# MegviiRobot/CamLaserCalibraTool

Measured on NVIDIA H100. Metric: residual+Jacobian evals/sec (full LM solves), higher is better.
Workload: dtype f64

## Files before the change

### camlasercalibratool_b200/_lib.py

```python
from __future__ import annotations

import ctypes as C
import os

from . import _build

c_double_p = C.POINTER(C.c_double)
c_int64_p = C.POINTER(C.c_int64)


class ClcError(RuntimeError):
    pass


class ProblemDesc(C.Structure):
    _fields_ = [
        ("n_frames", C.c_int64),
        ("frame_pose", c_double_p),
        ("offsets", c_int64_p),
        ("points", c_double_p),
        ("edge_points", c_double_p),
        ("use_loss", C.c_int),
        ("cauchy_a", C.c_double),
        ("device", C.c_int),
# ... 141 lines not shown
                                    C.POINTER(C.c_int32), C.POINTER(C.c_int32), C.c_int]),
    "clc_estimate_board_poses": (C.c_int, [C.POINTER(CameraDesc), C.c_int64, c_int64_p, C.POINTER(C.c_int32), C.POINTER(C.c_float),
                                           c_double_p, C.POINTER(C.c_int32), C.c_int]),
    "clc_T_to_pose7": (None, [c_double_p, c_double_p]),
    "clc_pose7_to_T": (None, [c_double_p, c_double_p]),
    "clc_shard_range": (C.c_int, [C.c_int64, c_int64_p, C.c_int, C.c_int, c_int64_p, c_int64_p]),
    "clc_comm_unique_id": (C.c_int, [_P]),
    "clc_comm_create": (C.c_int, [C.POINTER(_P), _P, C.c_int, C.c_int, C.c_int]),
    "clc_comm_destroy": (C.c_int, [_P]),
    "clc_comm_p2p_export": (C.c_int, [_P, _P]),
    "clc_comm_p2p_import": (C.c_int, [_P, _P]),
    "clc_problem_attach_comm": (C.c_int, [_P, _P]),
    "clc_problem_set_allreduce_mode": (C.c_int, [_P, C.c_int]),
    "clc_bench_eval": (C.c_int, [_P, c_double_p, C.c_int, C.c_int, C.POINTER(C.c_float)]),
    "clc_problem_algorithmic_bytes": (C.c_int, [_P, c_int64_p]),
    "clc_problem_streamed_bytes": (C.c_int, [_P, c_int64_p]),
    "clc_problem_set_planar_mode": (C.c_int, [_P, C.c_int]),
    "clc_debug_pack": (C.c_int, [C.c_int64, C.POINTER(c_double_p), c_int64_p, C.c_int64, C.c_int64, C.c_int, c_double_p,
                                 C.POINTER(C.c_int)]),
    "clc_debug_partition": (C.c_int, [_P, C.POINTER(C.c_int), c_int64_p, C.POINTER(C.c_int), C.POINTER(C.c_int),
                                      C.POINTER(C.c_int)]),
    "clc_debug_dispatch": (C.c_int, [_P, C.POINTER(C.c_int), C.POINTER(C.c_int), C.POINTER(C.c_int), C.POINTER(C.c_int),
                                     C.POINTER(C.c_int)]),
    "clc_bench_h2d": (C.c_int, [C.c_int64, C.c_int, C.c_int, C.POINTER(C.c_float)]),
    "clc_solve_readback_bytes": (C.c_int64, []),
    "clc_host_alloc": (C.c_int, [C.POINTER(_P), C.c_int64]),
    "clc_host_free": (C.c_int, [_P]),
    "clc_launch_count": (C.c_int64, []),
}

_lib = None


def lib_path() -> str:
    return _build.LIB_PATH


def load():
    global _lib
    if _lib is not None:
        return _lib
    path = os.environ.get("CLC_LIB_PATH", _build.LIB_PATH)
    if path == _build.LIB_PATH and _build.is_stale():
        try:
            _build.build()
        except Exception as exc:
# ... 19 lines not shown
```

### camlasercalibratool_b200/api.py

```python
from __future__ import annotations

import ctypes as C
from dataclasses import dataclass, field

import numpy as np

from . import _lib
from ._lib import ClcError, GatherDesc, LmIteration, LmOptions, LmSummary, ProblemDesc, SyntheticDesc, TERMINATION


def _dp(a):
    return a.ctypes.data_as(_lib.c_double_p) if a is not None else None


def _ip(a):
    return a.ctypes.data_as(_lib.c_int64_p) if a is not None else None


@dataclass
class Oberserve:

    tagPose_Qca: np.ndarray = field(default_factory=lambda: np.array([0.0, 0.0, 0.0, 1.0]))
    tagPose_tca: np.ndarray = field(default_factory=lambda: np.zeros(3))
    points: np.ndarray = field(default_factory=lambda: np.zeros((0, 3)))
# ... 59 lines not shown
    d.n_frames_total = int(n_frames_total)
    d.frame_begin = int(frame_begin)
    d.frame_end = int(n_frames_total if frame_end is None else frame_end)
    d.beams, d.seed, d.sigma = int(beams), int(seed), float(sigma)
    d.with_edges, d.use_loss, d.cauchy_a, d.device = int(bool(with_edges)), int(bool(use_loss)), float(cauchy_a), int(device)
    d.camera_model = {None: 0, "none": 0, "radtan": 1, "pinhole": 1, "equi": 2}[camera]
    if d.camera_model:
        k = CAMERA_DEFAULTS["radtan" if d.camera_model == 1 else "equi"] if intrinsics is None else intrinsics
        d.camera_intrinsics = (C.c_double * 8)(*[float(v) for v in k])
        d.pixel_sigma = float(pixel_sigma)
        d.image_width, d.image_height = int(image_size[0]), int(image_size[1])
        d.grid_rows, d.grid_cols, d.tag_size, d.tag_spacing = int(grid[0]), int(grid[1]), float(grid[2]), float(grid[3])
    return d


def default_options(**kw) -> LmOptions:
    o = LmOptions()
    _lib.load().clc_lm_default_options(C.byref(o))
    for k, v in kw.items():
        setattr(o, k, v)
    return o


class Problem:

    def __init__(self, handle):
        self._h = handle
        self._L = _lib.load()
        self._comm = None

    @classmethod
    def from_arrays(cls, frame_pose, offsets, points, edge_points=None, use_loss=True, cauchy_a=0.05, device=-1):
        L = _lib.load()
        frame_pose = np.ascontiguousarray(frame_pose, dtype=np.float64).reshape(-1, 7)
        offsets = np.ascontiguousarray(offsets, dtype=np.int64)
        points = np.ascontiguousarray(points, dtype=np.float64).reshape(-1, 3)
        if edge_points is not None:
            edge_points = np.ascontiguousarray(edge_points, dtype=np.float64).reshape(-1, 6)
            if edge_points.shape[0] != frame_pose.shape[0]:
                raise ValueError("edge_points must be [n_frames, 6]")
        if offsets.shape[0] != frame_pose.shape[0] + 1 or (offsets.size and offsets[-1] != points.shape[0]):
            raise ValueError("offsets do not match frame_pose / points")
        d = ProblemDesc()
        d.n_frames = frame_pose.shape[0]
        d.frame_pose, d.offsets, d.points, d.edge_points = _dp(frame_pose), _ip(offsets), _dp(points), _dp(edge_points)
        d.use_loss, d.cauchy_a, d.device = int(bool(use_loss)), float(cauchy_a), int(device)
# ... 55 lines not shown
        b = C.c_int64()
        _lib.check(self._L.clc_problem_streamed_bytes(self._h, C.byref(b)), "clc_problem_streamed_bytes")
        return b.value

    @property
    def planar(self):
        return self.streamed_bytes() != self.algorithmic_bytes()

    def set_planar_mode(self, mode):
        _lib.check(self._L.clc_problem_set_planar_mode(self._h, int(mode)), "clc_problem_set_planar_mode")

    def partition(self, warp_table=True):
        grid, per_warp, stage, resident = C.c_int(), C.c_int64(), C.c_int(), C.c_int()
        L = self._L
        _lib.check(L.clc_debug_partition(self._h, C.byref(grid), C.byref(per_warp), C.byref(stage), C.byref(resident), None),
                   "clc_debug_partition")
        out = dict(grid=grid.value, per_warp=per_warp.value, stage=stage.value, resident_chunks=resident.value)
        if warp_table:
            wff = np.empty(grid.value * 12, dtype=np.int32)
            _lib.check(L.clc_debug_partition(self._h, None, None, None, None, wff.ctypes.data_as(C.POINTER(C.c_int))),
                       "clc_debug_partition")
            out["warp_first_frame"] = wff
        return out

    def dispatch(self):
        paths = [C.c_int() for _ in range(4)]
        shape = (C.c_int * 3)()
        _lib.check(self._L.clc_debug_dispatch(self._h, *[C.byref(v) for v in paths], shape), "clc_debug_dispatch")
        out = {k: _lib.PATHS[v.value] for k, v in zip(("eval", "information", "closed_form", "solve"), paths)}
        out["small_shape"] = tuple(shape)
        return out

    def download(self):
        nf, npts, he = self.sizes()
        fp, off, pts = np.empty((nf, 7)), np.empty(nf + 1, dtype=np.int64), np.empty((npts, 3))
        edge = np.empty((nf, 6)) if he else None
        planes = np.empty((nf, 4))
        _lib.check(self._L.clc_problem_download(self._h, _dp(fp), _ip(off), _dp(pts), _dp(edge), _dp(planes)),
                   "clc_problem_download")
        return dict(frame_pose=fp, offsets=off, points=pts, edge_points=edge, planes=planes)

    def download_true_poses(self):
        fp = np.empty((self.sizes()[0], 7))
        _lib.check(self._L.clc_problem_download_true_poses(self._h, _dp(fp)), "clc_problem_download_true_poses")
        return fp

# ... 288 lines not shown
```

### camlasercalibratool_b200/csrc/clc_api.cu

```cuda
#include <cuda_runtime.h>
#include <dlfcn.h>
#include <nccl.h>

#include <algorithm>
#include <atomic>
#include <chrono>
#include <cstdio>
#include <cstdlib>
#include <cstring>
#include <mutex>
#include <string>
#include <vector>

#include "../../include/clc_b200.h"
#include "clc_kernels.cuh"
#include "clc_l2_plan.h"
#include "clc_linefit.cuh"
#include "clc_small.cuh"

namespace {

thread_local std::string g_last_error;
std::atomic<int64_t> g_launches{0};

// ... 200 lines not shown
  int64_t l2_bytes = 0;
  int grid = 0;
  int64_t n_frames = 0, n_points = 0, n_points_padded = 0, n_edges = 0;
  int use_loss = 1;
  double cauchy_a = 0.05;
  double *x = nullptr, *y = nullptr, *z = nullptr;
  void *xy_block = nullptr, *z_block = nullptr;
  double* frame_pose = nullptr;
  double* frame_pose_true = nullptr;
  double* plane = nullptr;
  int64_t* offsets = nullptr;
  int* warp_first_frame = nullptr;
  double* edge_plane = nullptr;
  double* edge_pt = nullptr;
  unsigned long long* partials_ll = nullptr;
  unsigned int* launch_seq = nullptr;
  unsigned long long* pose_ll = nullptr;
  double* sums = nullptr;
  double* pose = nullptr;
  clc::LmState* lm = nullptr;
  double* flush_buf = nullptr;
  int64_t flush_n = 0;
  unsigned long long* timing = nullptr;
  bool use_pdl = true;
  int64_t l2_persist_bytes = 0;
  bool l2_window_set = false;
  int64_t l2_resident_bytes = -1;
  int resident_chunks = 0;
  bool small_kernel = true;
  int loop_in_kernel = 1;
  PinnedBlock* pinned = nullptr;
  double* h_sums = nullptr;
  int* h_done = nullptr;
  clc::LmState* h_lm = nullptr;
  clc_comm* comm_obj = nullptr;
  ncclComm_t comm = nullptr;
  int nranks = 1, rank = 0;
  int* p2p_error = nullptr;
  int allreduce_mode = 0;
  int64_t per_warp = 0;
  int grid_full = 0;
  cudaEvent_t ev0 = nullptr, ev1 = nullptr;
  int* d_nonplanar = nullptr;
  bool z_all_zero = false;
  bool host_planarity_known = false;
  bool planar = false;
  int planar_mode = 1;
  int64_t planar_min_points = 0;
};

namespace {

clc::ProblemView make_view(const clc_problem* p) {
  clc::ProblemView v;
  v.x = p->x; v.y = p->y; v.z = p->z;
  v.plane = p->plane;
  v.offsets = p->offsets;
  v.warp_first_frame = p->warp_first_frame;
  v.edge_plane = p->edge_plane;
  v.edge_pt = p->edge_pt;
  v.n_frames = p->n_frames;
  v.n_points = p->n_points;
  v.n_edges = p->n_edges;
  v.per_warp = p->per_warp;
  v.resident_chunks = p->resident_chunks;
  v.a2 = p->cauchy_a * p->cauchy_a;
  v.inv_a2 = 1.0 / v.a2;
  return v;
}

int set_device(const clc_problem* p) {
  CLC_CUDA(cudaSetDevice(p->device));
  return CLC_OK;
}

int launch_sweep(clc_problem* p, int mode, bool loss, bool edges, const double* d_pose, const int* d_done,
                 clc::LmState* d_lm, bool collective = true, bool pdl = false, int loop_sweeps = 1, bool l2_hints = false) {
  clc::SweepArgs a;
  a.pose7 = d_pose;
  a.done = d_done;
  a.partials_ll = p->partials_ll;
  a.sums = p->sums;
  a.launch_seq = p->launch_seq;
  a.pose_ll = p->pose_ll;
  a.lm = d_lm;
  a.use_loss = loss ? 1 : 0;
  a.use_edges = edges ? 1 : 0;
  a.l2_hints = l2_hints ? 1 : 0;
  a.loop_sweeps = loop_sweeps;
  a.timing = p->timing;
  a.nranks = 1;
  a.rank = 0;
  a.seq_counter = nullptr;
  a.error = p->p2p_error;
  if (p->nranks > 1 && p->allreduce_mode == 1 && collective) {
    clc_comm* c = p->comm_obj;
    a.nranks = c->nranks;
    a.rank = c->rank;
    a.seq_counter = reinterpret_cast<unsigned long long*>(static_cast<char*>(c->p2p_block) + c->mailbox_bytes());
    for (int r = 0; r < c->nranks; ++r) a.peer_mailbox[r] = static_cast<unsigned long long*>(c->peer_block[r]);
  }
  const clc::ProblemView v = make_view(p);
  cudaLaunchConfig_t cfg = {};
  cfg.gridDim = dim3((unsigned)p->grid);
  cfg.blockDim = dim3(clc::kThreads);
  cfg.dynamicSmemBytes = clc::dyn_smem_bytes(p->planar);
  cfg.stream = p->stream;
  cudaLaunchAttribute attr[1];
  attr[0].id = cudaLaunchAttributeProgrammaticStreamSerialization;
  attr[0].val.programmaticStreamSerializationAllowed = pdl ? 1 : 0;
  cfg.attrs = attr;
  cfg.numAttrs = 1;
  cudaError_t le;
// ... 56 lines not shown
  p->grid = p->grid_full;
  {
    const int64_t stages = (p->n_points + chunk - 1) / chunk;
    const int64_t blocks_needed = std::max<int64_t>(1, (stages + clc::kWarps - 1) / clc::kWarps);
    if (blocks_needed < p->grid) p->grid = (int)blocks_needed;
    int64_t single_block_max = (int64_t)clc::kWarps * 8 * clc::kChunk;
    if (const char* env = std::getenv("CLC_SINGLE_BLOCK_MAX_POINTS")) single_block_max = std::atoll(env);
    if (p->n_points <= single_block_max) p->grid = 1;
  }
  const int64_t n_warps = (int64_t)p->grid * clc::kWarps;
  p->per_warp = std::max<int64_t>(chunk, round_up((p->n_points + n_warps - 1) / n_warps, chunk));
  if (p->warp_first_frame) CLC_CUDA(cudaFreeAsync(p->warp_first_frame, p->stream));
  if (p->partials_ll) CLC_CUDA(cudaFreeAsync(p->partials_ll, p->stream));
  p->warp_first_frame = nullptr;
  p->partials_ll = nullptr;
  CLC_CUDA(cudaMallocAsync(&p->warp_first_frame, sizeof(int) * n_warps, p->stream));
  const size_t ll_bytes = sizeof(unsigned long long) * 2 * (size_t)p->grid * clc::kMaxOut;
  CLC_CUDA(cudaMallocAsync(&p->partials_ll, ll_bytes, p->stream));
  {
    const int64_t stage_bytes = (int64_t)(p->planar ? 2 : 3) * chunk * 8;
    const bool latency_bound = p->n_points <= clc::kSmallMaxResiduals;
    const int64_t budget = p->l2_persist_bytes > 0 ? 0 : clc::l2_resident_budget(p->l2_bytes, p->l2_resident_bytes);
    p->resident_chunks = clc::l2_resident_chunks(budget, p->grid, clc::kWarps, p->per_warp / chunk, stage_bytes, latency_bound);
  }
  CLC_CUDA(cudaMemsetAsync(p->partials_ll, 0, ll_bytes, p->stream));
  const int threads = 256;
  const int blocks = (int)((n_warps + threads - 1) / threads);
  clc::clc_warp_table_kernel<<<blocks, threads, 0, p->stream>>>(p->offsets, p->n_frames, p->n_points, p->per_warp, n_warps,
                                                                p->warp_first_frame);
  CLC_LAUNCH_CHECK();
  return CLC_OK;
}

int finish_create(clc_problem* p) {
  const int threads = 256;
  if (p->n_frames > 0) {
    const int blocks = (int)((p->n_frames + threads - 1) / threads);
    clc::clc_planes_kernel<<<blocks, threads, 0, p->stream>>>(p->frame_pose, p->n_frames, p->plane, p->edge_plane);
    CLC_LAUNCH_CHECK();
  }
  static std::mutex cfg_mutex;
  static int cached_blocks_per_sm[64] = {};
  int blocks_per_sm = 0;
  {
    std::lock_guard<std::mutex> lock(cfg_mutex);
    if (p->device < 64) blocks_per_sm = cached_blocks_per_sm[p->device];
  }
  if (blocks_per_sm == 0) {
    int occ = 0, occ_min = 1 << 30;
    const void* variants[] = {
        (const void*)clc::clc_sweep_kernel<true, clc::kModeLM, false>,         (const void*)clc::clc_sweep_kernel<true, clc::kModeLM, true>,
        (const void*)clc::clc_sweep_kernel<false, clc::kModeLM, false>,        (const void*)clc::clc_sweep_kernel<false, clc::kModeLM, true>,
        (const void*)clc::clc_sweep_kernel<false, clc::kModeClosedForm, false>, (const void*)clc::clc_sweep_kernel<false, clc::kModeClosedForm, true>,
        (const void*)clc::clc_sweep_kernel<true, clc::kModeLM, false, true>,   (const void*)clc::clc_sweep_kernel<true, clc::kModeLM, true, true>,
        (const void*)clc::clc_sweep_kernel<false, clc::kModeLM, false, true>,  (const void*)clc::clc_sweep_kernel<false, clc::kModeLM, true, true>};
    for (int v = 0; v < 10; ++v) {
      const void* fn = variants[v];
      const int smem = clc::dyn_smem_bytes((v & 1) != 0);
      CLC_CUDA(cudaFuncSetAttribute(fn, cudaFuncAttributeMaxDynamicSharedMemorySize, smem));
      CLC_CUDA(cudaOccupancyMaxActiveBlocksPerMultiprocessor(&occ, fn, clc::kThreads, smem));
      occ_min = std::min(occ_min, occ);
    }
    if (occ_min < 1) return fail(CLC_ERR_CUDA, "the sweep kernel does not fit on this device");
    blocks_per_sm = std::max(1, std::min(occ_min, clc::kBlocksPerSM));
    if (const char* env = std::getenv("CLC_BLOCKS_PER_SM")) {
      const int v = std::atoi(env);
      if (v >= 1) blocks_per_sm = std::min(v, std::max(1, occ_min));
    }
    std::lock_guard<std::mutex> lock(cfg_mutex);
    if (p->device < 64) cached_blocks_per_sm[p->device] = blocks_per_sm;
  }
  p->grid_full = p->num_sms * blocks_per_sm;
  if (const char* env = std::getenv("CLC_PDL")) p->use_pdl = std::atoi(env) != 0;
  if (const char* env = std::getenv("CLC_LOOP_IN_KERNEL")) p->loop_in_kernel = std::atoi(env);
  if (const char* env = std::getenv("CLC_SMALL_KERNEL")) p->small_kernel = std::atoi(env) != 0;
  if (const char* env = std::getenv("CLC_L2_PERSIST_MB")) p->l2_persist_bytes = (int64_t)std::atoll(env) << 20;
  if (const char* env = std::getenv("CLC_L2_RESIDENT_MB")) p->l2_resident_bytes = std::max<int64_t>(0, (int64_t)std::atoll(env) << 20);
  CLC_CUDA(cudaMallocAsync(&p->sums, sizeof(double) * clc::kMaxOut, p->stream));
  CLC_CUDA(cudaMallocAsync(&p->pose, sizeof(double) * 8, p->stream));
  CLC_CUDA(cudaMallocAsync(&p->launch_seq, sizeof(unsigned int), p->stream));
  CLC_CUDA(cudaMallocAsync(&p->pose_ll, sizeof(unsigned long long) * 16, p->stream));
  CLC_CUDA(cudaMemsetAsync(p->pose_ll, 0, sizeof(unsigned long long) * 16, p->stream));
  CLC_CUDA(cudaMallocAsync(&p->lm, sizeof(clc::LmState), p->stream));
  CLC_CUDA(cudaMallocAsync(&p->p2p_error, sizeof(int), p->stream));
  CLC_CUDA(cudaMemsetAsync(p->p2p_error, 0, sizeof(int), p->stream));
  CLC_CUDA(cudaMemsetAsync(p->launch_seq, 0, sizeof(unsigned int), p->stream));
  CLC_CUDA(cudaMemsetAsync(p->sums, 0, sizeof(double) * clc::kMaxOut, p->stream));
  p->pinned = pinned_acquire();
  if (!p->pinned) return fail(CLC_ERR_CUDA, "cudaMallocHost failed");
  p->h_sums = p->pinned->sums;
  p->h_done = &p->pinned->done;
  p->h_lm = &p->pinned->lm;
  if (p->host_planarity_known) {
    CLC_CUDA(cudaStreamSynchronize(p->stream));
  } else {
    p->pinned->nonplanar = 1;
    CLC_CUDA(cudaMemcpyAsync(&p->pinned->nonplanar, p->d_nonplanar, sizeof(int), cudaMemcpyDeviceToHost, p->stream));
    CLC_CUDA(cudaStreamSynchronize(p->stream));
    p->z_all_zero = p->pinned->nonplanar == 0;
  }
// ... 595 lines not shown
  if (!p) return fail(CLC_ERR_INVALID, "NULL problem");
  int rc = eval_all(&p, 1, pose7, 1);
  if (rc != CLC_OK) return rc;
  information_post(p->h_sums, H36, b6, chi, sv6, V36);
  return CLC_OK;
}

int clc_closed_form(clc_problem* p, double Tlc[16], int* unobservable, double AtA81[81], double Atb9[9]) {
  if (!p || !Tlc) return fail(CLC_ERR_INVALID, "NULL argument");
  int rc = eval_all(&p, 1, nullptr, 2);
  if (rc != CLC_OK) return rc;
  closed_form_post(p->h_sums, Tlc, unobservable, AtA81, Atb9);
  return CLC_OK;
}


namespace {

struct SolveCtx {
  clc_lm_options opt;
  int max_sweeps = 0;
  int launched = 0;
  bool fused_update = true, loss = true, edges = false;
};

int l2_window(clc_problem* p, bool on) {
  if (p->l2_persist_bytes <= 0 || !p->xy_block) return CLC_OK;
  if (on == p->l2_window_set) return CLC_OK;
  cudaStreamAttrValue attr;
  std::memset(&attr, 0, sizeof(attr));
  if (on) {
    int max_persist = 0, max_window = 0;
    CLC_CUDA(cudaDeviceGetAttribute(&max_persist, cudaDevAttrMaxPersistingL2CacheSize, p->device));
    CLC_CUDA(cudaDeviceGetAttribute(&max_window, cudaDevAttrMaxAccessPolicyWindowSize, p->device));
    const size_t set_aside = (size_t)std::min<int64_t>(p->l2_persist_bytes, max_persist);
    if (set_aside == 0 || max_window <= 0) return CLC_OK;
    size_t cur = 0;
    CLC_CUDA(cudaDeviceGetLimit(&cur, cudaLimitPersistingL2CacheSize));
    if (cur < set_aside) CLC_CUDA(cudaDeviceSetLimit(cudaLimitPersistingL2CacheSize, set_aside));
    const size_t span = sizeof(double) * (size_t)(p->y - p->x) + sizeof(double) * (size_t)p->n_points;
    const size_t window = std::min(span, (size_t)max_window);
    attr.accessPolicyWindow.base_ptr = p->xy_block;
    attr.accessPolicyWindow.num_bytes = window;
    attr.accessPolicyWindow.hitRatio = (float)std::min(1.0, (double)set_aside / (double)window);
    attr.accessPolicyWindow.hitProp = cudaAccessPropertyPersisting;
    attr.accessPolicyWindow.missProp = cudaAccessPropertyStreaming;
// ... 20 lines not shown
  ctx->fused_update = fused_lm_update(p);
  ctx->loss = p->use_loss != 0;
  ctx->edges = p->n_edges > 0;
  ctx->max_sweeps = opt.max_num_iterations + 2;
  ctx->launched = 0;
  *p->h_done = 0;
  return CLC_OK;
}

int solve_launch_one(clc_problem* p, SolveCtx* ctx, int loop_sweeps = 1) {
  int rc = set_device(p);
  if (rc != CLC_OK) return rc;
  rc = launch_sweep(p, clc::kModeLM, ctx->loss, ctx->edges, p->lm->core.cand, &p->lm->core.done,
                    ctx->fused_update ? p->lm : nullptr, true, ctx->fused_update && p->use_pdl, loop_sweeps,
                    true);
  if (rc != CLC_OK) return rc;
  if (!ctx->fused_update) {
    rc = allreduce_sums(p, clc::kNumSums);
    if (rc != CLC_OK) return rc;
    clc::clc_lm_kernel<<<1, 32, 0, p->stream>>>(p->lm, p->sums);
    CLC_LAUNCH_CHECK();
  }
  ctx->launched++;
  return CLC_OK;
}

int solve_poll_enqueue(clc_problem* p) {
  int rc = set_device(p);
  if (rc != CLC_OK) return rc;
  CLC_CUDA(cudaMemcpyAsync(p->h_done, &p->lm->core.done, sizeof(int), cudaMemcpyDeviceToHost, p->stream));
  return CLC_OK;
}

int l2_demote(clc_problem* p) {
  if (p->resident_chunks == 0) return CLC_OK;
  int rc = set_device(p);
  if (rc != CLC_OK) return rc;
  const int chunk = p->planar ? clc::kPlanarChunk : clc::kChunk;
  const int64_t n_warps = (int64_t)p->grid * clc::kWarps;
  const int64_t lines = n_warps * p->resident_chunks * (chunk / 16);
  const int threads = 256;
  clc::clc_l2_demote_kernel<<<(unsigned)((lines + threads - 1) / threads), threads, 0, p->stream>>>(make_view(p), n_warps, chunk);
  CLC_LAUNCH_CHECK();
  return CLC_OK;
}

int solve_finish(clc_problem* p, double pose7[7], clc_lm_summary* summary, clc_lm_iteration* trace, int trace_cap) {
  int rc = l2_demote(p);
  if (rc != CLC_OK) return rc;
  CLC_CUDA(cudaEventRecord(p->ev1, p->stream));
  rc = l2_window(p, false);
  if (rc != CLC_OK) return rc;
  CLC_CUDA(cudaMemcpyAsync(p->h_lm, p->lm, sizeof(clc::LmState), cudaMemcpyDeviceToHost, p->stream));
  CLC_CUDA(sync_stream_low_latency(p->stream));
  float ms = 0.f;
  CLC_CUDA(cudaEventElapsedTime(&ms, p->ev0, p->ev1));
  rc = check_p2p_error(p);
  if (rc != CLC_OK) return rc;
  const clc::LmCore& s = p->h_lm->core;
  const clc_lm_iteration* dev_trace = p->h_lm->trace;
  if (pose7)
    for (int i = 0; i < 7; ++i) pose7[i] = s.x[i];
  if (summary) {
    summary->termination = s.done ? s.done : CLC_TERM_NO_CONVERGENCE;
    summary->num_iterations = s.n_trace;
    summary->num_successful_steps = s.num_successful;
    summary->num_unsuccessful_steps = s.num_unsuccessful;
    summary->num_sweeps = s.sweeps;
    summary->reserved = 0;
    summary->initial_cost = s.initial_cost;
    summary->final_cost = s.x_cost;
    summary->device_ms = ms;
  }
// ... 38 lines not shown
    launched = max_sweeps;
  }
  bool loop_launch = launched == 0;
  for (int g = 0; g < n; ++g)
    loop_launch = loop_launch && ctx[g].fused_update && sweep_loops_in_kernel(ps[g]);
  if (loop_launch) {
    for (int g = 0; g < n; ++g) {
      rc = solve_launch_one(ps[g], &ctx[g], max_sweeps);
      if (rc != CLC_OK) return rc;
    }
    launched = max_sweeps;
  }
  while (launched < max_sweeps) {
    const int batch = std::min(launched == 0 ? 2 * opt.iterations_per_sync : opt.iterations_per_sync, max_sweeps - launched);
    for (int i = 0; i < batch; ++i)
      for (int g = 0; g < n; ++g) {
        rc = solve_launch_one(ps[g], &ctx[g]);
        if (rc != CLC_OK) return rc;
      }
    launched += batch;
    for (int g = 0; g < n; ++g) {
      rc = solve_poll_enqueue(ps[g]);
      if (rc != CLC_OK) return rc;
    }
    bool all_done = true;
    for (int g = 0; g < n; ++g) {
      rc = set_device(ps[g]);
      if (rc != CLC_OK) return rc;
      CLC_CUDA(sync_stream_low_latency(ps[g]->stream));
      all_done = all_done && (*ps[g]->h_done != 0);
    }
    if (all_done) break;
  }
  demote_on_exit.armed = false;
  double ms_max = 0.0;
  int first_rc = CLC_OK;
  for (int g = n - 1; g >= 0; --g) {
    clc_lm_summary sg;
    rc = solve_finish(ps[g], g == 0 ? pose7 : nullptr, &sg, g == 0 ? trace : nullptr, trace_cap);
    if (rc != CLC_OK && first_rc == CLC_OK) first_rc = rc;
    if (rc == CLC_OK) {
      ms_max = std::max(ms_max, sg.device_ms);
      if (g == 0 && summary) *summary = sg;
    }
  }
  if (first_rc != CLC_OK) return first_rc;
  if (summary) summary->device_ms = ms_max;
  return CLC_OK;
}

}

int clc_solve_lm(clc_problem* p, double pose7[7], const clc_lm_options* opt_in, clc_lm_summary* summary,
                 clc_lm_iteration* trace, int trace_cap) {
  if (!p || !pose7) return fail(CLC_ERR_INVALID, "NULL argument");
  return solve_all(&p, 1, pose7, opt_in, summary, trace, trace_cap);
}


int clc_problem_line_fit(clc_problem* p, double* lines, int max_num_iterations, double* info) {
  if (!p || !lines || max_num_iterations < 0) return fail(CLC_ERR_INVALID, "bad line-fit arguments");
  int rc = set_device(p);
// ... 734 lines not shown
    }
    clc::clc_flush_kernel<<<p->num_sms * 4, 256, 0, p->stream>>>(p->flush_buf, p->flush_n, 1.0);
    CLC_LAUNCH_CHECK();
    clc::clc_flush_read_kernel<<<p->num_sms * 4, 256, 0, p->stream>>>(p->flush_buf, p->flush_n, p->flush_buf);
    CLC_LAUNCH_CHECK();
  }
  clc_lm_options opt;
  clc_lm_default_options(&opt);
  clc::lm_init(&p->h_lm->core, pose7, opt);
  CLC_CUDA(cudaMemcpyAsync(p->lm, p->h_lm, sizeof(clc::LmState), cudaMemcpyHostToDevice, p->stream));
  CLC_CUDA(cudaMemcpyAsync(p->pose, pose7, sizeof(double) * 7, cudaMemcpyHostToDevice, p->stream));
  rc = launch_sweep(p, clc::kModeLM, p->use_loss != 0, p->n_edges > 0, p->pose, nullptr, with_lm ? p->lm : nullptr, false);
  cudaError_t e = cudaMemcpyAsync(stamps, p->timing, bytes, cudaMemcpyDeviceToHost, p->stream);
  if (e == cudaSuccess && warp_stamps)
    e = cudaMemcpyAsync(warp_stamps, p->timing + 8 * (size_t)p->grid, wbytes, cudaMemcpyDeviceToHost, p->stream);
  if (e == cudaSuccess) e = cudaStreamSynchronize(p->stream);
  cudaFreeAsync(p->timing, p->stream);
  p->timing = nullptr;
  if (rc != CLC_OK) return rc;
  if (e != cudaSuccess) return fail(CLC_ERR_CUDA, cudaGetErrorString(e));
  return CLC_OK;
}

int clc_debug_lm_profile(long long out[16]) {
  if (!out) return fail(CLC_ERR_INVALID, "NULL argument");
  for (int i = 0; i < 16; ++i) out[i] = 0;
#ifdef CLC_LM_PROFILE
  CLC_CUDA(cudaMemcpyFromSymbol(out, clc::g_lm_profile, sizeof(long long) * 16));
#endif
  return CLC_OK;
}

int clc_bench_h2d(int64_t bytes, int device, int reps, float* ms_each) {
  if (bytes < 1 || reps < 1 || !ms_each) return fail(CLC_ERR_INVALID, "bad h2d bench arguments");
  if (device >= 0) CLC_CUDA(cudaSetDevice(device));
  void *h = nullptr, *d = nullptr;
  cudaStream_t st = nullptr;
  cudaEvent_t e0 = nullptr, e1 = nullptr;
  cudaError_t e = cudaHostAlloc(&h, (size_t)bytes, cudaHostAllocDefault);
  if (e == cudaSuccess) { std::memset(h, 0, (size_t)bytes); e = cudaMalloc(&d, (size_t)bytes); }
  if (e == cudaSuccess) e = cudaStreamCreateWithFlags(&st, cudaStreamNonBlocking);
  if (e == cudaSuccess) e = cudaEventCreate(&e0);
  if (e == cudaSuccess) e = cudaEventCreate(&e1);
  for (int i = -1; i < reps && e == cudaSuccess; ++i) {
    e = cudaEventRecord(e0, st);
    if (e == cudaSuccess) e = cudaMemcpyAsync(d, h, (size_t)bytes, cudaMemcpyHostToDevice, st);
// ... 28 lines not shown
```

### camlasercalibratool_b200/csrc/clc_kernels.cuh

```cuda
#pragma once

#include <cuda_runtime.h>

#include "clc_camera.cuh"
#include "clc_expand.cuh"
#include "clc_lm.cuh"

namespace clc {

#ifndef CLC_THREADS
#define CLC_THREADS 384
#endif
#ifndef CLC_BLOCKS_PER_SM
#define CLC_BLOCKS_PER_SM 1
#endif
#ifndef CLC_STAGES
#define CLC_STAGES 2
#endif
constexpr int kThreads = CLC_THREADS;
constexpr int kBlocksPerSM = CLC_BLOCKS_PER_SM;
constexpr int kWarps = kThreads / 32;
constexpr int kTileStride = 13;
#ifndef CLC_CHUNK
#define CLC_CHUNK 128
// ... 21 lines not shown
constexpr int kBarsPerWarp = kStages > kPlanarStages ? kStages : kPlanarStages;
constexpr int kTileDoublesPerWarp = 32 * kTileStride;
__host__ __device__ constexpr int ring_doubles_per_warp(bool planar) { return planar ? kPlanarStages * 2 * kPlanarChunk : kStages * 3 * kChunk; }
__host__ __device__ constexpr int dyn_smem_bytes(bool planar) {
  return kWarps * ring_doubles_per_warp(planar) * 8 + kWarps * kTileDoublesPerWarp * 8 + kWarps * kBarsPerWarp * 8;
}

enum SweepMode { kModeLM = 0, kModeClosedForm = 1 };

struct ProblemView {
  const double* x;
  const double* y;
  const double* z;
  const double* plane;
  const int64_t* offsets;
  const int* warp_first_frame;
  const double* edge_plane;
  const double* edge_pt;
  int64_t n_frames;
  int64_t n_points;
  int64_t n_edges;
  int64_t per_warp;
  int resident_chunks;
  double inv_a2;
  double a2;
};

struct SweepArgs {
  const double* pose7;
  const int* done;
  unsigned long long* partials_ll;
  double* sums;
  unsigned int* launch_seq;
  LmState* lm;
  int use_loss;
  int use_edges;
  int l2_hints;
  int loop_sweeps;
  unsigned long long* pose_ll;
  unsigned long long* timing;
  int nranks;
  int rank;
  unsigned long long* seq_counter;
  unsigned long long* peer_mailbox[kMaxRanks];
  int* error;
};


__device__ __forceinline__ unsigned long long globaltimer_ns() {
  unsigned long long t;
  asm volatile("mov.u64 %0, %globaltimer;" : "=l"(t));
  return t;
}
#define CLC_STAMP(slot)                                                                       \
  do {                                                                                        \
    if (args.timing != nullptr && threadIdx.x == 0) args.timing[(int64_t)blockIdx.x * 8 + (slot)] = globaltimer_ns(); \
  } while (0)

__device__ __forceinline__ uint32_t smem_u32(const void* p) { return (uint32_t)__cvta_generic_to_shared(p); }

// ... 7 lines not shown
  uint32_t done;
  do {
    asm volatile(
        "{\n\t.reg .pred p;\n\t"
        "mbarrier.try_wait.parity.shared::cta.b64 p, [%1], %2;\n\t"
        "selp.u32 %0, 1, 0, p;\n\t}"
        : "=r"(done)
        : "r"(smem_u32(bar)), "r"(parity)
        : "memory");
  } while (!done);
}
__device__ __forceinline__ void bulk_g2s(void* dst, const void* src, uint32_t bytes, uint64_t* bar) {
  asm volatile("cp.async.bulk.shared::cluster.global.mbarrier::complete_tx::bytes [%0], [%1], %2, [%3];" ::"r"(
                   smem_u32(dst)),
               "l"(src), "r"(bytes), "r"(smem_u32(bar))
               : "memory");
}
__device__ __forceinline__ void bulk_g2s_hint(void* dst, const void* src, uint32_t bytes, uint64_t* bar, uint64_t policy) {
  asm volatile("cp.async.bulk.shared::cluster.global.mbarrier::complete_tx::bytes.L2::cache_hint [%0], [%1], %2, [%3], %4;" ::"r"(
                   smem_u32(dst)),
               "l"(src), "r"(bytes), "r"(smem_u32(bar)), "l"(policy)
               : "memory");
}
__device__ __forceinline__ uint64_t policy_evict_last() {
  uint64_t pol;
  asm("createpolicy.fractional.L2::evict_last.b64 %0, 1.0;" : "=l"(pol));
  return pol;
}
__device__ __forceinline__ uint64_t policy_evict_first() {
  uint64_t pol;
  asm("createpolicy.fractional.L2::evict_first.b64 %0, 1.0;" : "=l"(pol));
  return pol;
}

__device__ __forceinline__ void st_relaxed_sys(unsigned long long* p, unsigned long long v) {
  asm volatile("st.relaxed.sys.global.u64 [%0], %1;" ::"l"(p), "l"(v) : "memory");
}
__device__ __forceinline__ unsigned long long ld_relaxed_sys(const unsigned long long* p) {
  unsigned long long v;
  asm volatile("ld.relaxed.sys.global.u64 %0, [%1];" : "=l"(v) : "l"(p) : "memory");
  return v;
}

__device__ __forceinline__ void st_volatile_v2(unsigned long long* p, unsigned long long a, unsigned long long b) {
  asm volatile("st.volatile.global.v2.u64 [%0], {%1, %2};" ::"l"(p), "l"(a), "l"(b) : "memory");
}
__device__ __forceinline__ void ld_volatile_v2(const unsigned long long* p, unsigned long long& a, unsigned long long& b) {
  asm volatile("ld.volatile.global.v2.u64 {%0, %1}, [%2];" : "=l"(a), "=l"(b) : "l"(p) : "memory");
}

__device__ __forceinline__ unsigned int ld_acquire_gpu(const unsigned int* p) {
  unsigned int v;
  asm volatile("ld.acquire.gpu.global.u32 %0, [%1];" : "=r"(v) : "l"(p) : "memory");
  return v;
}
__device__ __forceinline__ unsigned int atom_add_acq_rel_gpu(unsigned int* p, unsigned int v) {
  unsigned int old;
  asm volatile("atom.acq_rel.gpu.global.add.u32 %0, [%1], %2;" : "=r"(old) : "l"(p), "r"(v) : "memory");
  return old;
}

__device__ __forceinline__ double rcp_pos(double a) {
  double r;
  asm("rcp.approx.ftz.f64 %0, %1;" : "=d"(r) : "d"(a));
  double e = fma(-a, r, 1.0);
  r = fma(r, e, r);
  e = fma(-a, r, 1.0);
  r = fma(r, e, r);
  return r;
}

// ... 136 lines not shown
        bulk_g2s_hint(dst + CH, pv.y + src, CH * 8, bars + st, pol);
        if (!PLANAR) bulk_g2s_hint(dst + 2 * CH, pv.z + src, CH * 8, bars + st, pol);
      } else {
        bulk_g2s(dst, pv.x + src, CH * 8, bars + st);
        bulk_g2s(dst + CH, pv.y + src, CH * 8, bars + st);
        if (!PLANAR) bulk_g2s(dst + 2 * CH, pv.z + src, CH * 8, bars + st);
      }
    }
    ++issued;
    if (LOOP && ++next_c == n_chunks) next_c = 0;
  };
  auto drain = [&](int g) {
    for (; g < issued; ++g) mbar_wait(bars + g % NST, (uint32_t)(g / NST) & 1u);
  };
  if (lane == 0) {
#pragma unroll
    for (int st = 0; st < NST; ++st) mbar_init(bars + st, 1);
    asm volatile("fence.mbarrier_init.release.cluster;" ::: "memory");
    asm volatile("fence.proxy.async.shared::cta;" ::: "memory");
  }
  __syncwarp();
  for (int g = 0; g < NST && g < total_chunks; ++g) issue_one(false);
  __syncwarp();

  asm volatile("griddepcontrol.wait;" ::: "memory");
  if (args.done != nullptr && (*args.done != 0 || (args.error != nullptr && *args.error != 0))) {
    drain(0);
    return;
  }

  const unsigned int launch_tag0 = *args.launch_seq + 1u;
  if (MODE == kModeLM && args.lm != nullptr && blockIdx.x == 0) {
    const unsigned long long* g_core = reinterpret_cast<const unsigned long long*>(&args.lm->core);
    for (int k = threadIdx.x; k < kLmCoreWords; k += kThreads) s_core[k] = __ldcg(g_core + k);
  }

  PoseConsts pc;
  int n_tile = 0;

  auto flush_tile = [&]() {
    double out[NOUT];
#pragma unroll
    for (int k = 0; k < NOUT; ++k) out[k] = 0.0;
    __syncwarp();
    if (lane < n_tile) {
      const double* row = tile + lane * kTileStride;
      const int64_t f = __double_as_longlong(row[12]);
      double plane[4];
// ... 193 lines not shown
    if (__any_sync(0xffffffffu, any)) {
      double v[32];
#pragma unroll
      for (int k = 0; k < 32; ++k) v[k] = (k < NOUT) ? out[k] : 0.0;
      warp_transpose_sum<32>(v, lane);
      if (lane < NOUT) s_acc[warp][lane] += v[0];
      __syncwarp();
    }
  }

  const unsigned long long ll_tag = (unsigned long long)launch_tag << 32;
  __syncthreads();
  double block_sum = 0.0;
  if (threadIdx.x < NOUT) {
#pragma unroll
    for (int wv = 0; wv < kWarps; ++wv) block_sum += s_acc[wv][threadIdx.x];
    if (gridDim.x > 1) {
      const unsigned long long bits = (unsigned long long)__double_as_longlong(block_sum);
      st_volatile_v2(args.partials_ll + ((int64_t)blockIdx.x * kMaxOut + threadIdx.x) * 2, ll_tag | (bits & 0xffffffffull),
                     ll_tag | (bits >> 32));
    }
  }
  CLC_STAMP(3);
  asm volatile("griddepcontrol.launch_dependents;" ::: "memory");
  if (blockIdx.x != 0 && (!LOOP || sweeps_max == 1)) return;

  if (blockIdx.x == 0) {
    constexpr int PARTS = kThreads / NOUT;
    constexpr int NB = 10;
    double* s_gather = &s_red[0][0];
    static_assert(kWarps * 32 >= PARTS * NOUT, "s_red holds one value per gathering thread");
    if (gridDim.x > 1 && threadIdx.x < PARTS * NOUT) {
      const int k = threadIdx.x % NOUT, part = threadIdx.x / NOUT;
      double acc = 0.0;
      for (int base = part; base < (int)gridDim.x; base += PARTS * NB) {
        unsigned long long w0[NB], w1[NB];
        unsigned int pending = 0u;
#pragma unroll
        for (int u = 0; u < NB; ++u)
          if (base + u * PARTS < (int)gridDim.x) pending |= 1u << u;
        unsigned int polls = 0;
        unsigned long long t0 = 0;
        while (pending != 0u) {
#pragma unroll
          for (int u = 0; u < NB; ++u)
            if ((pending >> u) & 1u)
              ld_volatile_v2(args.partials_ll + ((int64_t)(base + u * PARTS) * kMaxOut + k) * 2, w0[u], w1[u]);
// ... 302 lines not shown
```

### camlasercalibratool_b200/csrc/clc_l2_plan.h

```cpp
#pragma once

#include <algorithm>
#include <cstdint>

namespace clc {

constexpr double kL2ResidentFraction = 0.5;

inline int64_t l2_resident_budget(int64_t l2_bytes, int64_t override_bytes) {
  return override_bytes >= 0 ? override_bytes : (int64_t)((double)l2_bytes * kL2ResidentFraction);
}

inline int l2_resident_chunks(int64_t budget_bytes, int64_t grid, int64_t warps_per_block, int64_t stages_per_warp,
                              int64_t stage_bytes, bool latency_bound) {
  if (budget_bytes <= 0 || grid <= 1 || latency_bound || stages_per_warp <= 0 || stage_bytes <= 0) return 0;
  return (int)std::min<int64_t>(stages_per_warp, budget_bytes / (grid * warps_per_block * stage_bytes));
}

}
```

### include/clc_b200.h

```cpp
#ifndef CLC_B200_H
#define CLC_B200_H

#include <stdint.h>

#ifdef __cplusplus
extern "C" {
#endif

#define CLC_OK 0
#define CLC_ERR_INVALID 1
#define CLC_ERR_CUDA 2
#define CLC_ERR_NCCL 3
#define CLC_ERR_STATE 4

typedef struct clc_problem clc_problem;

typedef struct {
  int64_t n_frames;
  const double* frame_pose;
  const int64_t* offsets;
  const double* points;
  const double* edge_points;
  int use_loss;
  double cauchy_a;
// ... 138 lines not shown
int clc_group_create_gather(clc_group** out, const clc_gather_desc* desc, const int* devices, int n_devices);
int clc_group_create_synthetic(clc_group** out, const clc_synthetic_desc* desc, const int* devices, int n_devices);
int clc_group_destroy(clc_group* g);
int clc_group_size(const clc_group* g, int* n_devices, int64_t* n_frames, int64_t* n_points);
int clc_group_problem(clc_group* g, int index, clc_problem** out);
int clc_group_eval(clc_group* g, const double pose7[7], double H36[36], double g6[6], double* cost);
int clc_group_solve_lm(clc_group* g, double pose7[7], const clc_lm_options* opt, clc_lm_summary* summary,
                       clc_lm_iteration* trace, int trace_cap);
int clc_group_information(clc_group* g, const double pose7[7], double H36[36], double b6[6], double* chi,
                          double singular_values6[6], double V36[36]);
int clc_group_closed_form(clc_group* g, double Tlc16[16], int* unobservable, double AtA81[81], double Atb9[9]);
int clc_default_devices(int* devices, int cap, int* n);

int clc_bench_eval(clc_problem* p, const double pose7[7], int n, int flush_l2, float* ms_each);
int clc_problem_algorithmic_bytes(const clc_problem* p, int64_t* bytes);
int clc_problem_streamed_bytes(const clc_problem* p, int64_t* bytes);
int clc_problem_set_planar_mode(clc_problem* p, int mode);
int clc_upload_last_stats(double* total_ms, double* pack_wait_ms, int64_t* bytes_h2d, int* chunks, int* pack_threads,
                          int* direct);
int clc_debug_pack(int64_t n_frames, const double* const* frame_points, const int64_t* frame_counts, int64_t a, int64_t b,
                   int xy, double* out, int* nonplanar);
int clc_debug_partition(const clc_problem* p, int* grid, int64_t* per_warp, int* stage_points, int* resident_chunks,
                        int* warp_first_frame);
#define CLC_PATH_ONE_CLUSTER 1
#define CLC_PATH_SINGLE_BLOCK 2
#define CLC_PATH_SINGLE_BLOCK_LOOP 3
#define CLC_PATH_MULTI_BLOCK 4
#define CLC_PATH_MULTI_BLOCK_LOOP 5
int clc_debug_dispatch(const clc_problem* p, int* eval_path, int* information_path, int* closed_form_path, int* solve_path,
                       int* small_shape);
int clc_bench_h2d(int64_t bytes, int device, int reps, float* ms_each);
int64_t clc_solve_readback_bytes(void);
int clc_host_alloc(void** ptr, int64_t bytes);
int clc_host_free(void* ptr);
int64_t clc_launch_count(void);

#ifdef __cplusplus
}
#endif
#endif
```

Baseline: 92.46 billion.

## Prefetch L2 head chunks and release PDL dependents early in LM sweep kernel

In the per-sweep LM kernel, each warp now issues bulk L2 prefetches for a head region of its upcoming point chunks (sized by an L2 budget fraction) before waiting on the prior grid. When only one block fits per SM, it also triggers griddepcontrol.launch_dependents early so the next sweep's prologue can overlap the current sweep's tail. The intent is to hide DRAM latency at sweep boundaries and shrink the gap between dependent launches. The cost is extra L2 pressure that may evict resident data. Per-slice timing instrumentation and debug APIs are added as well.

```diff
diff --git a/camlasercalibratool_b200/_lib.py b/camlasercalibratool_b200/_lib.py
--- a/camlasercalibratool_b200/_lib.py
+++ b/camlasercalibratool_b200/_lib.py
@@ -187,6 +187,9 @@
                                       C.POINTER(C.c_int)]),
     "clc_debug_dispatch": (C.c_int, [_P, C.POINTER(C.c_int), C.POINTER(C.c_int), C.POINTER(C.c_int), C.POINTER(C.c_int),
                                      C.POINTER(C.c_int)]),
+    "clc_debug_l2_head": (C.c_int, [_P, C.POINTER(C.c_int), C.POINTER(C.c_int)]),
+    "clc_debug_solve_timeline": (C.c_int, [_P, c_double_p, C.POINTER(LmOptions), C.POINTER(C.c_ulonglong), C.POINTER(C.c_ulonglong),
+                                           C.POINTER(C.c_int), C.POINTER(C.c_int), C.POINTER(LmSummary)]),
     "clc_bench_h2d": (C.c_int, [C.c_int64, C.c_int, C.c_int, C.POINTER(C.c_float)]),
     "clc_solve_readback_bytes": (C.c_int64, []),
     "clc_host_alloc": (C.c_int, [C.POINTER(_P), C.c_int64]),
diff --git a/camlasercalibratool_b200/api.py b/camlasercalibratool_b200/api.py
--- a/camlasercalibratool_b200/api.py
+++ b/camlasercalibratool_b200/api.py
@@ -105,6 +105,30 @@
     return o
 
 
+def sweep_timeline_table(stamps, warp_done=None):
+    st = np.asarray(stamps, dtype=np.int64)
+    rows = []
+    for i in range(st.shape[0]):
+        s = st[i]
+        real = bool(np.all(s[:, 1] > 0))
+        r = dict(real=real, stream=None, tail=None, gather=None, lm=None, boundary=None, period=None)
+        nxt = st[i + 1] if i + 1 < st.shape[0] else None
+        if nxt is not None:
+            r["period"] = (int(nxt[:, 6].min()) - int(s[:, 6].min())) * 1e-3
+        if real:
+            done = s[:, 1] if warp_done is None else np.asarray(warp_done[i], dtype=np.int64).reshape(st.shape[1], -1).max(axis=1)
+            med = float(np.median(done))
+            last_partial = int(s[:, 3].max())
+            r["stream"] = (med - int(s[:, 6].min())) * 1e-3
+            r["tail"] = (int(done.max()) - med) * 1e-3
+            r["gather"] = max(0, int(s[0, 4]) - last_partial) * 1e-3
+            r["lm"] = (int(s[0, 5]) - int(s[0, 4])) * 1e-3
+            if nxt is not None:
+                r["boundary"] = (int(nxt[:, 6].min()) - last_partial) * 1e-3
+        rows.append(r)
+    return rows
+
+
 class Problem:
 
     def __init__(self, handle):
@@ -206,6 +230,25 @@
                        "clc_debug_partition")
             out["warp_first_frame"] = wff
         return out
+
+    def l2_head(self):
+        head, early = C.c_int(), C.c_int()
+        _lib.check(self._L.clc_debug_l2_head(self._h, C.byref(head), C.byref(early)), "clc_debug_l2_head")
+        return dict(head_chunks=head.value, early_release=bool(early.value))
+
+    def solve_timeline(self, pose7, options: LmOptions | None = None):
+        x = np.ascontiguousarray(pose7, dtype=np.float64).copy()
+        o = options if options is not None else default_options()
+        slices = o.max_num_iterations + 2
+        grid = self.partition(warp_table=False)["grid"]
+        st = np.zeros((slices, grid, 8), dtype=np.uint64)
+        wd = np.zeros((slices, grid * 12), dtype=np.uint64)
+        g, n, s = C.c_int(), C.c_int(), LmSummary()
+        u64p = C.POINTER(C.c_ulonglong)
+        _lib.check(self._L.clc_debug_solve_timeline(self._h, _dp(x), C.byref(o), st.ctypes.data_as(u64p), wd.ctypes.data_as(u64p),
+                                                    C.byref(g), C.byref(n), C.byref(s)), "clc_debug_solve_timeline")
+        st, wd = st[:n.value].astype(np.int64), wd[:n.value].astype(np.int64)
+        return dict(stamps=st, warp_done=wd, summary=s, sweeps=sweep_timeline_table(st, wd))
 
     def dispatch(self):
         paths = [C.c_int() for _ in range(4)]
diff --git a/camlasercalibratool_b200/csrc/clc_api.cu b/camlasercalibratool_b200/csrc/clc_api.cu
--- a/camlasercalibratool_b200/csrc/clc_api.cu
+++ b/camlasercalibratool_b200/csrc/clc_api.cu
@@ -246,11 +246,16 @@
   double* flush_buf = nullptr;
   int64_t flush_n = 0;
   unsigned long long* timing = nullptr;
+  int timing_slices = 0;
+  int timing_used = 0;
   bool use_pdl = true;
   int64_t l2_persist_bytes = 0;
   bool l2_window_set = false;
   int64_t l2_resident_bytes = -1;
   int resident_chunks = 0;
+  int64_t l2_head_bytes = -1;
+  int head_chunks = 0;
+  bool early_release = true;
   bool small_kernel = true;
   int loop_in_kernel = 1;
   PinnedBlock* pinned = nullptr;
@@ -288,6 +293,7 @@
   v.n_edges = p->n_edges;
   v.per_warp = p->per_warp;
   v.resident_chunks = p->resident_chunks;
+  v.head_chunks = p->head_chunks;
   v.a2 = p->cauchy_a * p->cauchy_a;
   v.inv_a2 = 1.0 / v.a2;
   return v;
@@ -311,8 +317,13 @@
   a.use_loss = loss ? 1 : 0;
   a.use_edges = edges ? 1 : 0;
   a.l2_hints = l2_hints ? 1 : 0;
+  a.early_release = (pdl && p->early_release) ? 1 : 0;
   a.loop_sweeps = loop_sweeps;
   a.timing = p->timing;
+  if (p->timing_slices > 0) {
+    const size_t slice = (size_t)(8 + clc::kWarps) * (size_t)p->grid;
+    a.timing = p->timing_used < p->timing_slices ? p->timing + slice * (size_t)p->timing_used++ : nullptr;
+  }
   a.nranks = 1;
   a.rank = 0;
   a.seq_counter = nullptr;
@@ -415,6 +426,10 @@
     const bool latency_bound = p->n_points <= clc::kSmallMaxResiduals;
     const int64_t budget = p->l2_persist_bytes > 0 ? 0 : clc::l2_resident_budget(p->l2_bytes, p->l2_resident_bytes);
     p->resident_chunks = clc::l2_resident_chunks(budget, p->grid, clc::kWarps, p->per_warp / chunk, stage_bytes, latency_bound);
+    const int ring_stages = p->planar ? clc::kPlanarStages : clc::kStages;
+    const int64_t head_budget = p->l2_persist_bytes > 0 ? 0 : clc::l2_head_budget(p->l2_bytes, p->l2_head_bytes);
+    p->head_chunks = clc::l2_head_chunks(head_budget, p->grid, clc::kWarps, p->per_warp / chunk, stage_bytes, ring_stages,
+                                         p->resident_chunks, latency_bound);
   }
   CLC_CUDA(cudaMemsetAsync(p->partials_ll, 0, ll_bytes, p->stream));
   const int threads = 256;
@@ -434,10 +449,14 @@
   }
   static std::mutex cfg_mutex;
   static int cached_blocks_per_sm[64] = {};
-  int blocks_per_sm = 0;
+  static int cached_occ_max[64] = {};
+  int blocks_per_sm = 0, occ_max = 0;
   {
     std::lock_guard<std::mutex> lock(cfg_mutex);
-    if (p->device < 64) blocks_per_sm = cached_blocks_per_sm[p->device];
+    if (p->device < 64) {
+      blocks_per_sm = cached_blocks_per_sm[p->device];
+      occ_max = cached_occ_max[p->device];
+    }
   }
   if (blocks_per_sm == 0) {
     int occ = 0, occ_min = 1 << 30;
@@ -453,6 +472,7 @@
       CLC_CUDA(cudaFuncSetAttribute(fn, cudaFuncAttributeMaxDynamicSharedMemorySize, smem));
       CLC_CUDA(cudaOccupancyMaxActiveBlocksPerMultiprocessor(&occ, fn, clc::kThreads, smem));
       occ_min = std::min(occ_min, occ);
+      occ_max = std::max(occ_max, occ);
     }
     if (occ_min < 1) return fail(CLC_ERR_CUDA, "the sweep kernel does not fit on this device");
     blocks_per_sm = std::max(1, std::min(occ_min, clc::kBlocksPerSM));
@@ -461,14 +481,20 @@
       if (v >= 1) blocks_per_sm = std::min(v, std::max(1, occ_min));
     }
     std::lock_guard<std::mutex> lock(cfg_mutex);
-    if (p->device < 64) cached_blocks_per_sm[p->device] = blocks_per_sm;
+    if (p->device < 64) {
+      cached_blocks_per_sm[p->device] = blocks_per_sm;
+      cached_occ_max[p->device] = occ_max;
+    }
   }
   p->grid_full = p->num_sms * blocks_per_sm;
   if (const char* env = std::getenv("CLC_PDL")) p->use_pdl = std::atoi(env) != 0;
+  p->early_release = blocks_per_sm == 1 && occ_max == 1;
+  if (const char* env = std::getenv("CLC_PDL_EARLY")) p->early_release = p->early_release && std::atoi(env) != 0;
   if (const char* env = std::getenv("CLC_LOOP_IN_KERNEL")) p->loop_in_kernel = std::atoi(env);
   if (const char* env = std::getenv("CLC_SMALL_KERNEL")) p->small_kernel = std::atoi(env) != 0;
   if (const char* env = std::getenv("CLC_L2_PERSIST_MB")) p->l2_persist_bytes = (int64_t)std::atoll(env) << 20;
   if (const char* env = std::getenv("CLC_L2_RESIDENT_MB")) p->l2_resident_bytes = std::max<int64_t>(0, (int64_t)std::atoll(env) << 20);
+  if (const char* env = std::getenv("CLC_L2_HEAD_MB")) p->l2_head_bytes = std::max<int64_t>(0, (int64_t)std::atoll(env) << 20);
   CLC_CUDA(cudaMallocAsync(&p->sums, sizeof(double) * clc::kMaxOut, p->stream));
   CLC_CUDA(cudaMallocAsync(&p->pose, sizeof(double) * 8, p->stream));
   CLC_CUDA(cudaMallocAsync(&p->launch_seq, sizeof(unsigned int), p->stream));
@@ -1110,6 +1136,7 @@
   int max_sweeps = 0;
   int launched = 0;
   bool fused_update = true, loss = true, edges = false;
+  bool end_enqueued = false;
 };
 
 int l2_window(clc_problem* p, bool on) {
@@ -1176,6 +1203,7 @@
     CLC_LAUNCH_CHECK();
   }
   ctx->launched++;
+  ctx->end_enqueued = false;
   return CLC_OK;
 }
 
@@ -1199,10 +1227,17 @@
   return CLC_OK;
 }
 
-int solve_finish(clc_problem* p, double pose7[7], clc_lm_summary* summary, clc_lm_iteration* trace, int trace_cap) {
+int solve_end_enqueue(clc_problem* p, SolveCtx* ctx) {
   int rc = l2_demote(p);
   if (rc != CLC_OK) return rc;
   CLC_CUDA(cudaEventRecord(p->ev1, p->stream));
+  ctx->end_enqueued = true;
+  return CLC_OK;
+}
+
+int solve_finish(clc_problem* p, SolveCtx* ctx, double pose7[7], clc_lm_summary* summary, clc_lm_iteration* trace, int trace_cap) {
+  int rc = ctx->end_enqueued ? CLC_OK : solve_end_enqueue(p, ctx);
+  if (rc != CLC_OK) return rc;
   rc = l2_window(p, false);
   if (rc != CLC_OK) return rc;
   CLC_CUDA(cudaMemcpyAsync(p->h_lm, p->lm, sizeof(clc::LmState), cudaMemcpyDeviceToHost, p->stream));
@@ -1287,6 +1322,8 @@
     for (int g = 0; g < n; ++g) {
       rc = solve_poll_enqueue(ps[g]);
       if (rc != CLC_OK) return rc;
+      rc = solve_end_enqueue(ps[g], &ctx[g]);
+      if (rc != CLC_OK) return rc;
     }
     bool all_done = true;
     for (int g = 0; g < n; ++g) {
@@ -1302,7 +1339,7 @@
   int first_rc = CLC_OK;
   for (int g = n - 1; g >= 0; --g) {
     clc_lm_summary sg;
-    rc = solve_finish(ps[g], g == 0 ? pose7 : nullptr, &sg, g == 0 ? trace : nullptr, trace_cap);
+    rc = solve_finish(ps[g], &ctx[g], g == 0 ? pose7 : nullptr, &sg, g == 0 ? trace : nullptr, trace_cap);
     if (rc != CLC_OK && first_rc == CLC_OK) first_rc = rc;
     if (rc == CLC_OK) {
       ms_max = std::max(ms_max, sg.device_ms);
@@ -2083,6 +2120,49 @@
   return CLC_OK;
 }
 
+int clc_debug_solve_timeline(clc_problem* p, const double pose7[7], const clc_lm_options* opt_in, unsigned long long* stamps,
+                             unsigned long long* warp_stamps, int* grid_out, int* launches, clc_lm_summary* summary) {
+  if (!p || !pose7 || !stamps) return fail(CLC_ERR_INVALID, "bad timeline arguments");
+  clc_lm_options opt;
+  if (opt_in) opt = *opt_in; else clc_lm_default_options(&opt);
+  if (opt.max_num_iterations < 0) return fail(CLC_ERR_INVALID, "max_num_iterations < 0");
+  int rc = set_device(p);
+  if (rc != CLC_OK) return rc;
+  if (grid_out) *grid_out = p->grid;
+  const int slices = opt.max_num_iterations + 2;
+  const size_t slice = (size_t)(8 + clc::kWarps) * (size_t)p->grid;
+  const size_t bytes = sizeof(unsigned long long) * slice * (size_t)slices;
+  CLC_CUDA(cudaMallocAsync(&p->timing, bytes, p->stream));
+  CLC_CUDA(cudaMemsetAsync(p->timing, 0, bytes, p->stream));
+  p->timing_slices = slices;
+  p->timing_used = 0;
+  double x[7];
+  for (int i = 0; i < 7; ++i) x[i] = pose7[i];
+  rc = solve_all(&p, 1, x, &opt, summary, nullptr, 0);
+  if (launches) *launches = p->timing_used;
+  p->timing_slices = 0;
+  std::vector<unsigned long long> h(slice * (size_t)slices);
+  cudaError_t e = cudaMemcpyAsync(h.data(), p->timing, bytes, cudaMemcpyDeviceToHost, p->stream);
+  if (e == cudaSuccess) e = cudaStreamSynchronize(p->stream);
+  cudaFreeAsync(p->timing, p->stream);
+  p->timing = nullptr;
+  if (rc != CLC_OK) return rc;
+  if (e != cudaSuccess) return fail(CLC_ERR_CUDA, cudaGetErrorString(e));
+  const size_t blk = 8 * (size_t)p->grid, wrp = (size_t)clc::kWarps * (size_t)p->grid;
+  for (int s = 0; s < slices; ++s) {
+    std::memcpy(stamps + blk * s, h.data() + slice * s, sizeof(unsigned long long) * blk);
+    if (warp_stamps) std::memcpy(warp_stamps + wrp * s, h.data() + slice * s + blk, sizeof(unsigned long long) * wrp);
+  }
+  return CLC_OK;
+}
+
+int clc_debug_l2_head(const clc_problem* p, int* head_chunks, int* early_release) {
+  if (!p) return fail(CLC_ERR_INVALID, "NULL problem");
+  if (head_chunks) *head_chunks = p->head_chunks;
+  if (early_release) *early_release = p->early_release ? 1 : 0;
+  return CLC_OK;
+}
+
 int clc_debug_lm_profile(long long out[16]) {
   if (!out) return fail(CLC_ERR_INVALID, "NULL argument");
   for (int i = 0; i < 16; ++i) out[i] = 0;
diff --git a/camlasercalibratool_b200/csrc/clc_kernels.cuh b/camlasercalibratool_b200/csrc/clc_kernels.cuh
--- a/camlasercalibratool_b200/csrc/clc_kernels.cuh
+++ b/camlasercalibratool_b200/csrc/clc_kernels.cuh
@@ -67,6 +67,7 @@
   int64_t n_edges;
   int64_t per_warp;
   int resident_chunks;
+  int head_chunks;
   double inv_a2;
   double a2;
 };
@@ -81,6 +82,7 @@
   int use_loss;
   int use_edges;
   int l2_hints;
+  int early_release;
   int loop_sweeps;
   unsigned long long* pose_ll;
   unsigned long long* timing;
@@ -134,6 +136,9 @@
                "l"(src), "r"(bytes), "r"(smem_u32(bar)), "l"(policy)
                : "memory");
 }
+__device__ __forceinline__ void prefetch_l2(const void* src, uint32_t bytes) {
+  asm volatile("cp.async.bulk.prefetch.L2.global [%0], %1;" ::"l"(src), "r"(bytes) : "memory");
+}
 __device__ __forceinline__ uint64_t policy_evict_last() {
   uint64_t pol;
   asm("createpolicy.fractional.L2::evict_last.b64 %0, 1.0;" : "=l"(pol));
@@ -159,6 +164,12 @@
 }
 __device__ __forceinline__ void ld_volatile_v2(const unsigned long long* p, unsigned long long& a, unsigned long long& b) {
   asm volatile("ld.volatile.global.v2.u64 {%0, %1}, [%2];" : "=l"(a), "=l"(b) : "l"(p) : "memory");
+}
+
+__device__ __forceinline__ int ld_relaxed_gpu(const int* p) {
+  int v;
+  asm volatile("ld.relaxed.gpu.global.s32 %0, [%1];" : "=r"(v) : "l"(p) : "memory");
+  return v;
 }
 
 __device__ __forceinline__ unsigned int ld_acquire_gpu(const unsigned int* p) {
@@ -341,8 +352,21 @@
   __syncwarp();
   for (int g = 0; g < NST && g < total_chunks; ++g) issue_one(false);
   __syncwarp();
+  if (!LOOP && MODE == kModeLM) {
+    const int head_end = min(NST + pv.head_chunks, n_chunks - pv.resident_chunks);
+    if (args.l2_hints != 0 && lane == 0 && head_end > NST &&
+        (args.done == nullptr || ld_relaxed_gpu(args.done) == 0)) {
+      const int64_t src = p0 + (int64_t)NST * CH;
+      const uint32_t bytes = (uint32_t)(head_end - NST) * CH * 8;
+      prefetch_l2(pv.x + src, bytes);
+      prefetch_l2(pv.y + src, bytes);
+      if (!PLANAR) prefetch_l2(pv.z + src, bytes);
+    }
+    if (args.early_release != 0) asm volatile("griddepcontrol.launch_dependents;" ::: "memory");
+  }
 
   asm volatile("griddepcontrol.wait;" ::: "memory");
+  if (!LOOP) CLC_STAMP(6);
   if (args.done != nullptr && (*args.done != 0 || (args.error != nullptr && *args.error != 0))) {
     drain(0);
     return;
@@ -582,7 +606,7 @@
     }
   }
   CLC_STAMP(3);
-  asm volatile("griddepcontrol.launch_dependents;" ::: "memory");
+  if (LOOP || MODE != kModeLM || args.early_release == 0) asm volatile("griddepcontrol.launch_dependents;" ::: "memory");
   if (blockIdx.x != 0 && (!LOOP || sweeps_max == 1)) return;
 
   if (blockIdx.x == 0) {
diff --git a/camlasercalibratool_b200/csrc/clc_l2_plan.h b/camlasercalibratool_b200/csrc/clc_l2_plan.h
--- a/camlasercalibratool_b200/csrc/clc_l2_plan.h
+++ b/camlasercalibratool_b200/csrc/clc_l2_plan.h
@@ -17,4 +17,18 @@
   return (int)std::min<int64_t>(stages_per_warp, budget_bytes / (grid * warps_per_block * stage_bytes));
 }
 
+constexpr double kL2HeadFraction = 0.15;
+
+inline int64_t l2_head_budget(int64_t l2_bytes, int64_t override_bytes) {
+  return override_bytes >= 0 ? override_bytes : (int64_t)((double)l2_bytes * kL2HeadFraction);
 }
+
+inline int l2_head_chunks(int64_t budget_bytes, int64_t grid, int64_t warps_per_block, int64_t stages_per_warp,
+                          int64_t stage_bytes, int64_t ring_stages, int64_t resident_chunks, bool latency_bound) {
+  if (budget_bytes <= 0 || grid <= 1 || latency_bound || stages_per_warp <= 0 || stage_bytes <= 0) return 0;
+  const int64_t room = stages_per_warp - ring_stages - resident_chunks;
+  if (room <= 0) return 0;
+  return (int)std::min<int64_t>(room, budget_bytes / (grid * warps_per_block * stage_bytes));
+}
+
+}
diff --git a/include/clc_b200.h b/include/clc_b200.h
--- a/include/clc_b200.h
+++ b/include/clc_b200.h
@@ -184,6 +184,9 @@
                    int xy, double* out, int* nonplanar);
 int clc_debug_partition(const clc_problem* p, int* grid, int64_t* per_warp, int* stage_points, int* resident_chunks,
                         int* warp_first_frame);
+int clc_debug_l2_head(const clc_problem* p, int* head_chunks, int* early_release);
+int clc_debug_solve_timeline(clc_problem* p, const double pose7[7], const clc_lm_options* opt, unsigned long long* stamps,
+                             unsigned long long* warp_stamps, int* grid, int* launches, clc_lm_summary* summary);
 #define CLC_PATH_ONE_CLUSTER 1
 #define CLC_PATH_SINGLE_BLOCK 2
 #define CLC_PATH_SINGLE_BLOCK_LOOP 3
```

New measurement: 93.86 billion (median of 6 runs). 1.02x the previous value.
